# ywz978020607/MASIC

Measured on AMD Instinct MI355X. Metric: stereo pairs/sec (enc+dec), higher is better.
Workload: dtype bf16; 1 GPU; HSIC(N=128,M=192,K=5) eval forward (enc+dec both views), 8x3x512x512 stereo pairs per GPU (BASELINE.json configs[1] shape), inputs resident in HBM (the graph's static input buffers); the device homography of batch k+1 is handed over with batch k (one-batch look-ahead of a loader): its device->host read, the float32 host chain and the upload of the sampling matrices are done every step, under the r; pairs_per_gpu=8, height=512, width=512, parallelism=dp1 (pairs sharded, no data-path collective)

## Files before the change

coremasic/mywork/MASIC.py:

```python
import math
import os

import numpy as np

import torch
import torch.nn as nn
import torch.nn.functional as F

from compressai.entropy_models import (EntropyBottleneck, GaussianConditional, GaussianMixtureConditional,
                                       GaussianMixtureConditional_gf)
from compressai.layers import GDN, MaskedConv2d, ResidualBlock, conv3x3
from compressai.models.utils import conv, deconv, update_registered_buffers
from masic_amd import ops as _hip
from masic_amd.homography import warp_matrices as _warp_matrices
from masic_amd import autograd as _ag
from masic_amd.streams import ForkJoin as _ForkJoin
from masic_amd import fp8 as _fp8
from masic_amd import deconv as _deconv
from masic_amd.f16k import F16K as _F16K, F8K as _F8K

_RELU, _LEAKY, _NONE = _hip.ACT_RELU, _hip.ACT_LEAKY, _hip.ACT_NONE
_CAT_F16K = True
_HEADS_GROUPED = True


class CompressionModel(nn.Module):

    def __init__(self, entropy_bottleneck_channels, init_weights=True):
        super().__init__()
        self.entropy_bottleneck1 = EntropyBottleneck(entropy_bottleneck_channels)
        self.entropy_bottleneck2 = EntropyBottleneck(entropy_bottleneck_channels)
        if init_weights:
            self._initialize_weights()

    def aux_loss(self):
        return sum(m.loss() for m in self.modules() if isinstance(m, EntropyBottleneck))

    def _initialize_weights(self):
        for m in self.modules():
            if isinstance(m, (nn.Conv2d, nn.ConvTranspose2d)):
                nn.init.kaiming_normal_(m.weight)
                if m.bias is not None:
                    nn.init.zeros_(m.bias)

    def forward(self, *args):
        raise NotImplementedError()

    def parameters(self):
        for child in self.children():
            if not isinstance(child, EntropyBottleneck):
                yield from child.parameters()

    def aux_parameters(self):
        for child in self.children():
            if isinstance(child, EntropyBottleneck):
                yield from child.parameters()

    def update(self, force=False):
        for child in self.children():
            if isinstance(child, EntropyBottleneck):
                child.update(force=force)


class RateDistortionLoss(nn.Module):

    def __init__(self, lmbda=1e-2):
        super().__init__()
        self.lmbda = lmbda

    def forward(self, output, target):
        N, _, H, W = target.size()
        n = N * H * W
        bpp = sum(_hip.sum_log(l.contiguous()) for l in output["likelihoods"].values()) / (-math.log(2) * n)
        mse = _hip.sse(output["x_hat"].contiguous(), target.contiguous()) / target.numel()
        return {"bpp_loss": bpp.float(), "mse_loss": mse.float(), "loss": (self.lmbda * 255 ** 2 * mse + bpp).float()}


class AverageMeter:
    def __init__(self):
        self.val = self.avg = self.sum = self.count = 0

    def update(self, val, n=1):
        self.val = val
        self.sum += val * n
        self.count += n
        self.avg = self.sum / self.count


_SIDE_STREAMS = {}


def _side_streams(device, n=4):
    key = torch.device(device).index
    pool = _SIDE_STREAMS.get(key)
    if pool is None:
        pool, seen = [], set()
        for _ in range(64):
            s = torch.cuda.Stream(device=device)
            if s.cuda_stream not in seen:
                seen.add(s.cuda_stream)
                pool.append(s)
            if len(pool) == n + 1:
                break
        pool = _SIDE_STREAMS[key] = tuple(pool)
    cur = torch.cuda.current_stream(device).cuda_stream
    return tuple(s for s in pool if s.cuda_stream != cur)[:n]


_TRAIN_STREAMS = os.environ.get("MASIC_TRAIN_STREAMS", "1") != "0"


def _keep_until(t, stream):
    if not (torch.is_tensor(t) or isinstance(t, _F16K)):
        return
    if not torch.cuda.is_current_stream_capturing():
        t.record_stream(stream)


def _bf16_inference(*tensors):
    from masic_amd import nn as _mnn
    if not _mnn.reduced_precision():
        return False
    return not (torch.is_grad_enabled() and any(t.requires_grad for t in tensors))


def _f16k_chain(convs, acts, x, in_op=0, out=None, out_coff=0, gate=None, gate_c=0):
    B, _, H, W = x.shape
    hw = (H, W)
    for cv in convs:
        if not cv.f16k_supported(B, *hw):
            return None
        hw = cv.out_hw(*hw)
    t = x if isinstance(x, _F16K) else _F16K.from_nchw(x, in_op=in_op)
    for cv, act in zip(convs[:-1], acts):
        t = cv.run_f16k(t, act=act)
    return convs[-1].run_f16k(t, act=acts[-1], want_nchw=out is None, out=out, out_coff=out_coff, gate=gate, gate_c=gate_c)


def _pair_conv(conv, xa, xb, gdn_in=None, gdn_out=None):
    B, _, H, W = xa.shape
    desc = conv._desc((B, 6, H, W))
    def g(m):
        return None if m is None else (m.beta.detach(), m.gamma.detach().contiguous(), m.inverse)
    bm = (gdn_in or gdn_out).beta_min if (gdn_in or gdn_out) is not None else 1e-6
    return _hip.conv5s1_pair(xa, xb, conv.packed_weight(desc), None if conv.bias is None else conv.bias.detach(),
                             gdn_in=g(gdn_in), gdn_out=g(gdn_out), beta_min=bm)


def _gdn_f16k(gdn, x):
    return _hip.gdn_f16k(x, gdn.beta.detach(), gdn.gamma.detach(), inverse=gdn.inverse, beta_min=gdn.beta_min)


def _analysis_f16k(owner, x, layouts=None):
    from masic_amd import nn as _mnn
    convs = (owner.g_a_conv1, owner.g_a_conv2, owner.g_a_conv3, owner.g_a_conv4)
    gdns = (owner.g_a_gdn1, owner.g_a_gdn2, owner.g_a_gdn3)
    B, C, H, W = x.shape
    c1 = convs[0]
    if (C, c1.out_channels, tuple(c1.kernel_size), tuple(c1.stride), tuple(c1.padding)) != (3, 128, (5, 5), (2, 2), (2, 2)):
        return None
    sizes = [((H - 1) // 2 + 1, (W - 1) // 2 + 1)]
    for cv in convs[1:]:
        if not cv.f16k_supported(B, *sizes[-1]):
            return None
        sizes.append(cv.out_hw(*sizes[-1]))
    if convs[1].out_channels != 128 or convs[2].out_channels != 128:
        return None
    b1 = None if c1.bias is None else c1.bias.detach()
    sc = _fp8.scales(owner)
    if layouts is not None and (sc is not None or _mnn._FP8 or _fp8.recording() or not convs[3].f16k_multi_supported(B, *sizes[2])):
        return None
    if sc is not None and convs[1].f8k_supported(B, *sizes[0]) and convs[2].f8k_supported(B, *sizes[1]):
        t8 = _hip.conv_a_gdn_f8k(x, c1.packed_first_layer_weight(), b1, (_mnn.packed_gdn_f16k(gdns[0]), gdns[0].inverse), sc["a1"])[0]
        t = convs[1].run_f8k(_F8K(t8, B, 128, *sizes[0], sc["a1"]), gdn=gdns[1], out="f8k", out_scale=sc["a2"])
        t = convs[2].run_f8k(t, gdn=gdns[2], out="f16k")
        return convs[3].run_f16k(t, want_nchw=True)
    t = _F16K(_hip.conv_a_gdn_f16k(x, c1.packed_first_layer_weight(), b1, (_mnn.packed_gdn_f16k(gdns[0]), gdns[0].inverse))[0], B, 128, *sizes[0], 128, 0)
    _fp8.record(owner, "a1", t.buf)
    t = convs[1].run_f16k(t, gdn=gdns[1])
    _fp8.record(owner, "a2", t.buf)
    t = convs[2].run_f16k(t, gdn=gdns[2])
    if layouts is not None:
        return convs[3].run_f16k_multi(t, **layouts)
    return convs[3].run_f16k(t, want_nchw=True)


class encode_hyper(nn.Module):

    def __init__(self, N, M):
        super().__init__()
        self.encode_hyper = nn.Sequential(
            conv(M, N, kernel_size=5, stride=1), nn.ReLU(inplace=True),
            conv(N, N, kernel_size=5), nn.ReLU(inplace=True),
            conv(N, N, kernel_size=5))

    def forward(self, y, abs16=None):
        s = self.encode_hyper
        if _bf16_inference(y, s[0].weight):
            z = _f16k_chain((s[0], s[2], s[4]), (_RELU, _RELU, _NONE), y if abs16 is None else abs16, in_op=_hip.INOP_ABS)
            if z is not None:
                return z
        t = s[0].run(y, in_op=_hip.INOP_ABS, act=_RELU)
        t = s[2].run(t, act=_RELU)
        return s[4].run(t)


class _GmmHeads(nn.Module):

    def _branch(self, seq, x, acts):
        t = seq[0].run(x, act=acts[0])
        t = seq[2].run(t, act=acts[1])
        return seq[4].run(t, act=acts[2])

    def _branch_f16k(self, seq, x, acts):
        t, (B, _, H, W) = x.buf, x.shape
        for i, (layer, act) in enumerate(zip((seq[0], seq[2], seq[4]), acts)):
            last = i == 2
            if layer.in_channels % 16 == 0 and layer.out_channels % 32 == 0:
                t = _hip.gemm_f16k(t, layer.packed_gemm_dma_weight(), layer.bias.detach(), B, layer.in_channels, layer.out_channels,
                                   H, W, act, want_nchw=last)
            else:
                t = _hip.gemm1x1_bf16(t, layer.packed_gemm_weight(), layer.bias.detach(), B, layer.in_channels, layer.out_channels,
                                      H, W, act, want_nchw=last)
        return t

    def _branch_f8k(self, seq, x, sc, tag, acts):
        l0, l1, l2 = seq[0], seq[2], seq[4]
        x8, (B, _, H, W) = x.buf, x.shape
        wp, ws = l0.packed_gemm_f8k_weight(sc["c"])
        t = _hip.gemm_f8k(x8, wp, ws, l0.bias.detach(), B, l0.in_channels, l0.out_channels, H, W, acts[0], out="f8k", out_scale=sc[tag])
        wp, ws = l1.packed_gemm_f8k_weight(sc[tag])
        t = _hip.gemm_f8k(t, wp, ws, l1.bias.detach(), B, l1.in_channels, l1.out_channels, H, W, acts[1], out="f16k")
        return _hip.gemm_f16k(t, l2.packed_gemm_dma_weight(), l2.bias.detach(), B, l2.in_channels, l2.out_channels, H, W, acts[2], want_nchw=True)

    _STACKS = (("gmm_sigma", "h_sigma", (_RELU, _RELU, _RELU)), ("gmm_means", "h_means", (_LEAKY, _LEAKY, _NONE)),
               ("gmm_weights", "h_weights", (_LEAKY, _LEAKY, _NONE)))

    def _grouped_heads_ok(self):
        return all(getattr(self, n)[i].in_channels % 16 == 0 and getattr(self, n)[i].out_channels % 32 == 0
                   for n, _, _ in self._STACKS for i in (0, 2, 4))

    def _heads_grouped(self, x, sc):
        B, _, H, W = x.shape
        t = [x.buf] * 3
        for i in range(3):
            layers = []
            for k, (name, tag, acts) in enumerate(self._STACKS):
                layer = getattr(self, name)[2 * i]
                L = dict(x=t[k], bias=layer.bias.detach(), Cin=layer.in_channels, Cout=layer.out_channels, act=acts[i],
                         out="nchw" if i == 2 else "f16k")
                if sc is not None and i < 2:
                    L["wp"], L["ws"] = layer.packed_gemm_f8k_weight(sc["c"] if i == 0 else sc[tag])
                    if i == 0:
                        L["out"], L["out_scale"] = "f8k", sc[tag]
                else:
                    L["wp"] = layer.packed_gemm_dma_weight()
                layers.append(L)
            t = _hip.gemm_f16k_group(layers, B, H, W)
        return tuple(t)

    def _f8k_heads_ok(self):
        return all(seq[i].in_channels % 32 == 0 and seq[i].out_channels % 32 == 0 for seq in (self.gmm_sigma, self.gmm_means, self.gmm_weights) for i in (0, 2)) \
            and all(seq[4].in_channels % 16 == 0 and seq[4].out_channels % 32 == 0 for seq in (self.gmm_sigma, self.gmm_means, self.gmm_weights))

    def heads(self, x, parallel=True):
        from masic_amd import nn as _mnn
        if isinstance(x, _F16K):
            if not x.whole:
                raise RuntimeError(f"_GmmHeads.heads: the grouped GEMMs read a whole buffer, not {x!r}")
            return self._heads_grouped(x, None)
        if _mnn.reduced_precision() and not (torch.is_grad_enabled() and (x.requires_grad or self.gmm_sigma[0].weight.requires_grad)):
            B, _, H, W = x.shape
            sc = _fp8.scales(self)
            use_f8 = sc is not None and self._f8k_heads_ok()
            if use_f8:
                xv = _F8K(_hip.nchw_to_f8k(x, sc["c"]), *x.shape, sc["c"])
                branch = lambda seq, tag, acts: self._branch_f8k(seq, xv, sc, tag, acts)
            else:
                xv = _F16K.from_nchw(x)
                xf = xv.buf

                def branch(seq, tag, acts):
                    if _fp8.recording():
                        _fp8.record(self, "c", x)
                        l0 = seq[0]
                        _fp8.record(self, tag, _hip.gemm_f16k(xf, l0.packed_gemm_dma_weight(), l0.bias.detach(), B, l0.in_channels, l0.out_channels, H, W, acts[0])
                                    if l0.in_channels % 16 == 0 and l0.out_channels % 32 == 0 else
                                    _hip.gemm1x1_bf16(xf, l0.packed_gemm_weight(), l0.bias.detach(), B, l0.in_channels, l0.out_channels, H, W, acts[0]))
                    return self._branch_f16k(seq, xv, acts)
            if _HEADS_GROUPED and not _fp8.recording() and self._grouped_heads_ok():
                return self._heads_grouped(xv, sc if use_f8 else None)
            if not parallel:
                return (branch(self.gmm_sigma, "h_sigma", (_RELU, _RELU, _RELU)),
                        branch(self.gmm_means, "h_means", (_LEAKY, _LEAKY, _NONE)),
                        branch(self.gmm_weights, "h_weights", (_LEAKY, _LEAKY, _NONE)))
            fj = _ForkJoin()
            cur = fj.main
            side = _side_streams(x.device)[2:4]
            outs = [None, None, None]
            for i, (st, (seq, tag, acts)) in enumerate(zip(side, ((self.gmm_means, "h_means", (_LEAKY, _LEAKY, _NONE)),
                                                                  (self.gmm_weights, "h_weights", (_LEAKY, _LEAKY, _NONE))))):
                fj.fork(st)
                with fj.on(st):
                    outs[i + 1] = branch(seq, tag, acts)
            outs[0] = branch(self.gmm_sigma, "h_sigma", (_RELU, _RELU, _RELU))
            for st in side:
                fj.join(st)
            for t in outs[1:] + [xv.buf]:
                _keep_until(t, cur)
            return tuple(outs)
        if torch.is_grad_enabled() and _ag.gmm_heads_supported(self, x):
            return _ag.gmm_heads(self, x)
        sigma = self._branch(self.gmm_sigma, x, (_RELU, _RELU, _RELU))
        means = self._branch(self.gmm_means, x, (_LEAKY, _LEAKY, _NONE))
        logits = self._branch(self.gmm_weights, x, (_LEAKY, _LEAKY, _NONE))
        return sigma, means, logits

    def forward(self, x):
        sigma, means, logits = self.heads(x)
        return sigma, means, _hip.softmax_k(logits, self.K)


class gmm_hyper_y1_same_resolution(_GmmHeads):

    def __init__(self, N, M, K):
        super().__init__()
        self.N, self.M, self.K = N, M, K
        self.gmm_sigma = nn.Sequential(
            deconv(4 * M, 6 * M, kernel_size=1, stride=1), nn.ReLU(inplace=True),
            deconv(6 * M, 4 * M, kernel_size=1, stride=1), nn.ReLU(inplace=True),
            conv(4 * M, M * K, kernel_size=1, stride=1), nn.ReLU(inplace=True))
        self.gmm_means = nn.Sequential(
            deconv(4 * M, 6 * M, kernel_size=1, stride=1), nn.LeakyReLU(inplace=True),
            deconv(6 * M, 4 * M, kernel_size=1, stride=1), nn.LeakyReLU(inplace=True),
            conv(4 * M, M * K, kernel_size=1, stride=1))
        self.gmm_weights = nn.Sequential(
            deconv(4 * M, 6 * M, kernel_size=1, stride=1), nn.LeakyReLU(inplace=True),
            deconv(6 * M, M * K, kernel_size=1, stride=1), nn.LeakyReLU(inplace=True),
            conv(M * K, M * K, kernel_size=1, stride=1))


class gmm_hyper_y2_same_resolution(_GmmHeads):

    def __init__(self, N, M, K):
        super().__init__()
        self.N, self.M, self.K = N, M, K
        self.gmm_sigma = nn.Sequential(
            conv(5 * M, 6 * M, kernel_size=1, stride=1), nn.ReLU(inplace=True),
            conv(6 * M, 4 * M, kernel_size=1, stride=1), nn.ReLU(inplace=True),
            conv(4 * M, M * K, kernel_size=1, stride=1), nn.ReLU(inplace=True))
        self.gmm_means = nn.Sequential(
            conv(5 * M, 6 * M, kernel_size=1, stride=1), nn.LeakyReLU(inplace=True),
            conv(6 * M, 4 * M, kernel_size=1, stride=1), nn.LeakyReLU(inplace=True),
            conv(4 * M, M * K, kernel_size=1, stride=1))
        self.gmm_weights = nn.Sequential(
            conv(5 * M, 6 * M, kernel_size=1, stride=1), nn.LeakyReLU(inplace=True),
            conv(6 * M, M * K, kernel_size=1, stride=1), nn.LeakyReLU(inplace=True),
            conv(M * K, M * K, kernel_size=1, stride=1))


class mask2weights(nn.Module):

    def __init__(self, N, M, Kw):
        super().__init__()
        self.maskconv = nn.Sequential(
            conv(1, 3, kernel_size=3, stride=2), nn.ReLU(inplace=True),
            conv(3, 6, kernel_size=3), nn.ReLU(inplace=True),
            conv(6, 6, kernel_size=3), nn.ReLU(inplace=True),
            conv(6, 3, kernel_size=3))
        self.N, self.M, self.Kw = N, M, Kw

    def forward(self, m):
        s = self.maskconv
        t = s[0].run(m, act=_RELU)
        t = s[2].run(t, act=_RELU)
        t = s[4].run(t, act=_RELU)
        return s[6].run(t, act=_hip.ACT_SOFTMAX_C)


def _synthesis_f16k(dec, y_hat):
    B, _, H, W = y_hat.shape
    convs = (dec.g_s_conv1, dec.g_s_conv2, dec.g_s_conv3)
    gdns = (dec.g_s_gdn1, dec.g_s_gdn2, dec.g_s_gdn3)
    sizes = [(H, W)]
    for cv in convs:
        if cv.out_channels != 128 or not cv.f16k_supported(B, *sizes[-1]):
            return None
        sizes.append(cv.out_hw(*sizes[-1]))
    if not dec.g_s_conv4.d2s_supported(B, *sizes[3]):
        return None
    t = y_hat if isinstance(y_hat, _F16K) else _F16K.from_nchw(y_hat)
    sc = _fp8.scales(dec)
    if sc is not None and convs[1].f8k_supported(B, *sizes[1]) and convs[2].f8k_supported(B, *sizes[2]):
        t = convs[0].run_f16k_f8out(t, sc["d1"], gdn=gdns[0])
        t = convs[1].run_f8k(t, gdn=gdns[1], out="f8k", out_scale=sc["d2"])
        t = convs[2].run_f8k(t, gdn=gdns[2], out="f16k")
        return dec.g_s_conv4.run_f16k_d2s(t)
    for i in range(3):
        if t.whole and _deconv.supported(convs[i], gdns[i], B, t.H, t.W):
            t = _deconv.run(convs[i], gdns[i], t)
        else:
            t = convs[i].run_f16k(t, gdn=gdns[i])
        if i < 2:
            _fp8.record(dec, "d%d" % (i + 1), t.buf)
    return dec.g_s_conv4.run_f16k_d2s(t)


class Encoder1(nn.Module):

    def __init__(self, N, M, **kwargs):
        super().__init__()
        self.g_a_conv1 = conv(3, N)
        self.g_a_gdn1 = GDN(N)
        self.g_a_conv2 = conv(N, N)
        self.g_a_gdn2 = GDN(N)
        self.g_a_conv3 = conv(N, N)
        self.g_a_gdn3 = GDN(N)
        self.g_a_conv4 = conv(N, M)

    def forward(self, x):
        g1 = self.g_a_gdn1(self.g_a_conv1(x))
        g2 = self.g_a_gdn2(self.g_a_conv2(g1))
        g3 = self.g_a_gdn3(self.g_a_conv3(g2))
        return self.g_a_conv4(g3), g1, g2, g3

    def latent(self, x):
        if _bf16_inference(x, self.g_a_conv1.weight):
            y = _analysis_f16k(self, x.contiguous())
            if y is not None:
                return y
        return self.forward(x)[0]

    def latent_layouts(self, x, **layouts):
        if _bf16_inference(x, self.g_a_conv1.weight):
            return _analysis_f16k(self, x.contiguous(), layouts=layouts)
        return None

    def latent_train(self, x):
        if _ag.analysis_supported(self, x):
            return _ag.analysis(self, x)
        return self.forward(x)[0]


class Decoder1(nn.Module):

    def __init__(self, N, M, **kwargs):
        super().__init__()
        self.g_s_conv1 = deconv(M, N)
        self.g_s_gdn1 = GDN(N, inverse=True)
        self.g_s_conv2 = deconv(N, N)
        self.g_s_gdn2 = GDN(N, inverse=True)
        self.g_s_conv3 = deconv(N, N)
        self.g_s_gdn3 = GDN(N, inverse=True)
        self.g_s_conv4 = deconv(N, 3)

    def forward(self, y_hat):
        g1 = self.g_s_gdn1(self.g_s_conv1(y_hat))
        g2 = self.g_s_gdn2(self.g_s_conv2(g1))
        g3 = self.g_s_gdn3(self.g_s_conv3(g2))
        return self.g_s_conv4(g3), g1, g2, g3

    def reconstruct(self, y_hat):
        if isinstance(y_hat, _F16K):
            return _synthesis_f16k(self, y_hat) if _bf16_inference(self.g_s_conv1.weight) else None
        if _bf16_inference(y_hat, self.g_s_conv1.weight):
            x_hat = _synthesis_f16k(self, y_hat)
            if x_hat is not None:
                return x_hat
        return self.forward(y_hat)[0]

    def reconstruct_train(self, y_hat):
        if _ag.synthesis_supported(self, y_hat):
            return _ag.synthesis(self, y_hat)
        return self.forward(y_hat)[0]


class Encoder2(nn.Module):

    def __init__(self, N, M, **kwargs):
        super().__init__()
        self.pre_conv = conv(6, 3, stride=1)
        self.pre_gdn = GDN(3)
        self.g_a_conv1 = conv(3, N)
        self.g_a_gdn1 = GDN(N)
# ... 927 lines not shown
```

Measured before the change: 4415 stereo pairs/s.

## Add dedicated stride-2 128->128 5x5 conv+GDN kernel for encoder layers 2-3

Adds a specialized HIP kernel for the 128-channel 5x5 stride-2 conv fused with GDN. It splits waves into weight-DMA and patch-DMA roles, keeps a ring buffer of weight slabs in LDS, double-buffers input patches, and prefetches gamma for an in-register GDN epilogue. It also maps images to XCDs when the batch is divisible by 8. The encoder chain routes its two middle layers through this kernel when supported, aiming to hide load latency behind MFMA. The cost is a large, shape-specialized kernel with one block per CU, which limits occupancy.

```diff
diff --git a/coremasic/mywork/MASIC.py b/coremasic/mywork/MASIC.py
--- a/coremasic/mywork/MASIC.py
+++ b/coremasic/mywork/MASIC.py
@@ -17,6 +17,7 @@
 from masic_amd.streams import ForkJoin as _ForkJoin
 from masic_amd import fp8 as _fp8
 from masic_amd import deconv as _deconv
+from masic_amd import conv_s2 as _conv_s2
 from masic_amd.f16k import F16K as _F16K, F8K as _F8K
 
 _RELU, _LEAKY, _NONE = _hip.ACT_RELU, _hip.ACT_LEAKY, _hip.ACT_NONE
@@ -177,9 +178,13 @@
         return convs[3].run_f16k(t, want_nchw=True)
     t = _F16K(_hip.conv_a_gdn_f16k(x, c1.packed_first_layer_weight(), b1, (_mnn.packed_gdn_f16k(gdns[0]), gdns[0].inverse))[0], B, 128, *sizes[0], 128, 0)
     _fp8.record(owner, "a1", t.buf)
-    t = convs[1].run_f16k(t, gdn=gdns[1])
-    _fp8.record(owner, "a2", t.buf)
-    t = convs[2].run_f16k(t, gdn=gdns[2])
+    for i in (1, 2):
+        if t.whole and _conv_s2.supported(convs[i], gdns[i], B, t.H, t.W):
+            t = _conv_s2.run(convs[i], gdns[i], t)
+        else:
+            t = convs[i].run_f16k(t, gdn=gdns[i])
+        if i == 1:
+            _fp8.record(owner, "a2", t.buf)
     if layouts is not None:
         return convs[3].run_f16k_multi(t, **layouts)
     return convs[3].run_f16k(t, want_nchw=True)
diff --git a/include/masic_conv_s2.h b/include/masic_conv_s2.h
--- /dev/null
+++ b/include/masic_conv_s2.h
@@ -0,0 +1,21 @@
+#ifndef MASIC_CONV_S2_H
+#define MASIC_CONV_S2_H
+
+#include <stddef.h>
+
+#ifdef __cplusplus
+extern "C" {
+#endif
+
+int masic_conv_s2_gdn_f16k_supported(int B, int Hi, int Wi);
+
+int masic_conv_s2_gdn_f16k_fwd(const void* x_f16k, const void* w_packed, const float* bias, const void* gdn_packed, void* y_f16k,
+                               int B, int Hi, int Wi, void* stream);
+
+int masic_conv_s2_gdn_f16k_kernel_name(int B, int Hi, int Wi, char* buf, size_t n);
+
+#ifdef __cplusplus
+}
+#endif
+
+#endif
diff --git a/masic_amd/conv_s2.py b/masic_amd/conv_s2.py
--- /dev/null
+++ b/masic_amd/conv_s2.py
@@ -0,0 +1,96 @@
+import ctypes
+import os
+
+import torch
+
+from . import _lib, ops
+from .f16k import F16K
+from .ops import _p, _stream
+
+HEADER_PATH = os.path.join(os.path.dirname(_lib.HEADER_PATH), "masic_conv_s2.h")
+CHANNELS = 128
+PACKED_BYTES = 8 * 5 * 20480
+
+
+def _bind():
+    if not os.path.exists(HEADER_PATH):
+        raise ImportError(f"masic_amd.conv_s2: {HEADER_PATH} is missing: the binding is derived from it.  There is no CPU fallback for "
+                          "the HIP path.")
+    with open(HEADER_PATH) as f:
+        signatures, constants, structs = _lib.parse_header(f.read(), header="masic_conv_s2.h")
+    if constants or structs:
+        raise ValueError("masic_conv_s2.h: declares constants or structs; it holds prototypes only")
+    for name, (res, args) in signatures.items():
+        if not name.startswith("masic_conv_s2_") or name in _lib.SIGNATURES:
+            raise ValueError(f"masic_conv_s2.h: {name} is not a masic_conv_s2_* entry point of its own")
+        fn = getattr(_lib.lib, name)
+        fn.restype = res
+        fn.argtypes = args
+    return signatures
+
+
+SIGNATURES = _bind()
+
+
+def out_hw(Hi, Wi):
+    return (Hi - 1) // 2 + 1, (Wi - 1) // 2 + 1
+
+
+def kernel_name(B, Hi, Wi):
+    buf = ctypes.create_string_buffer(96)
+    _lib.check(_lib.lib.masic_conv_s2_gdn_f16k_kernel_name(B, Hi, Wi, buf, 96), "conv_s2_gdn_f16k_kernel_name")
+    return buf.value.decode()
+
+
+def conv_s2_gdn_f16k(x16, packed, bias, gdn_packed, B, Hi, Wi, out16=None):
+    if x16.dtype != torch.int16 or not x16.is_cuda or x16.numel() != B * CHANNELS * Hi * Wi:
+        raise RuntimeError(f"masic_amd.conv_s2_gdn_f16k: input must be an F16K int16 CUDA buffer of [{B},{CHANNELS},{Hi},{Wi}]")
+    if packed.dtype != torch.int16 or packed.numel() * 2 != PACKED_BYTES or packed.device != x16.device:
+        raise RuntimeError("masic_amd.conv_s2_gdn_f16k: `packed` is not the slab stream of a 128 -> 128 5x5 stride-2 layer")
+    if gdn_packed.numel() * gdn_packed.element_size() != ops._int_query("masic_gdn_f16k_packed_bytes") or gdn_packed.device != x16.device:
+        raise RuntimeError("masic_amd.conv_s2_gdn_f16k: `gdn_packed` is not a packed 128-channel GDN")
+    if bias is not None:
+        ops._dev(bias, "bias")
+        if bias.numel() != CHANNELS or bias.device != x16.device:
+            raise RuntimeError("masic_amd.conv_s2_gdn_f16k: bias must hold 128 values on the input's device")
+    if not _lib.lib.masic_conv_s2_gdn_f16k_supported(B, Hi, Wi):
+        raise RuntimeError(f"masic_amd.conv_s2_gdn_f16k: shape [{B},{CHANNELS},{Hi},{Wi}] is not supported")
+    Ho, Wo = out_hw(Hi, Wi)
+    n_out = B * CHANNELS * Ho * Wo
+    if out16 is None:
+        out16 = torch.empty(n_out, dtype=torch.int16, device=x16.device)
+    elif out16.dtype != torch.int16 or out16.numel() != n_out or out16.device != x16.device or not out16.is_contiguous():
+        raise RuntimeError("masic_amd.conv_s2_gdn_f16k: out16 does not match the output")
+    timed = None
+    if ops._timer is not None:
+        desc = ops.make_conv_desc(B, CHANNELS, Hi, Wi, CHANNELS, 5, 5, 2, 2, prec=_lib.PREC_BF16)
+        timed = ops._timer_open(desc, lambda d, buf, n: _lib.lib.masic_conv_s2_gdn_f16k_kernel_name(B, Hi, Wi, buf, n))
+    _lib.check(_lib.lib.masic_conv_s2_gdn_f16k_fwd(_p(x16), _p(packed), _p(bias), _p(gdn_packed), _p(out16), B, Hi, Wi, _stream()),
+               "conv_s2_gdn_f16k_fwd")
+    if timed is not None:
+        ops._timer_close(timed)
+    return out16
+
+
+def supported(cv, gdn, B, Hi, Wi, out_ctot=None, out_coff=0, in_ctot=None, in_coff=0, y_pre=None, prec=_lib.PREC_BF16, products=None):
+    if gdn is None or getattr(cv, "transposed_conv", True) or getattr(cv, "masked_conv", True):
+        return False
+    if cv.in_channels != CHANNELS or cv.out_channels != CHANNELS:
+        return False
+    if cv._geometry() != (5, 5, 2, 2) or gdn.inverse or gdn.beta.numel() != CHANNELS:
+        return False
+    if prec != _lib.PREC_BF16 or y_pre is not None or (ops._gdn_flags(False, products) & 2):
+        return False
+    if out_coff != 0 or out_ctot not in (None, CHANNELS) or in_coff != 0 or in_ctot not in (None, CHANNELS):
+        return False
+    return bool(_lib.lib.masic_conv_s2_gdn_f16k_supported(B, Hi, Wi)) and cv.f16k_supported(B, Hi, Wi)
+
+
+def run(cv, gdn, x):
+    from .nn import packed_gdn_f16k
+    if not x.whole or x.C != CHANNELS:
+        raise RuntimeError(f"masic_amd.conv_s2.run: the kernel takes whole 128-channel tensors, not {x!r}")
+    desc = cv._desc_f16k(x.B, x.H, x.W, out_ctot=CHANNELS)
+    bias = None if cv.bias is None else cv.bias.detach()
+    y16 = conv_s2_gdn_f16k(x.buf, cv.packed_f16k_weight(desc), bias, packed_gdn_f16k(gdn), x.B, x.H, x.W)
+    return F16K(y16, x.B, CHANNELS, desc.Ho, desc.Wo, CHANNELS, 0)
diff --git a/masic_amd/csrc/conv_s2_gdn.hip b/masic_amd/csrc/conv_s2_gdn.hip
--- /dev/null
+++ b/masic_amd/csrc/conv_s2_gdn.hip
@@ -0,0 +1,236 @@
+#include "f16k_device.h"
+#include "masic_conv_s2.h"
+
+namespace {
+
+struct ConvS2Args {
+    const unsigned short* x;
+    const unsigned char* w;
+    const float* bias;
+    const unsigned char* gdn;
+    unsigned short* y;
+    int Hi, Wi, Ho, Wo, tiles_w, ntiles, xcd_images;
+};
+
+constexpr int CS_T = 5, CS_D = 2, CS_NWS = CS_D + 1, CS_WST = CS_T * 4096;
+constexpr int CS_CHUNKS = 8, CS_STEPS = CS_CHUNKS * 5;
+constexpr int CS_TH = 8, CS_TW = 32;
+constexpr int CS_PH = (CS_TH - 1) * 2 + 5, CS_PW = (CS_TW - 1) * 2 + 5, CS_PWH = (CS_PW + 1) / 2;
+constexpr int CS_HALF = CS_PH * CS_PWH;
+constexpr int CS_NPIX = (2 * CS_HALF + 31) / 32 * 32;
+constexpr int CS_NINSTR = CS_NPIX / 32;
+constexpr int CS_PB = CS_NINSTR * 1024;
+constexpr int CS_PSP = 6, CS_NPI = 2 * CS_PSP;
+constexpr int CS_RING = 0, CS_PATCH0 = CS_RING + CS_NWS * CS_WST, CS_BETA = CS_PATCH0 + 2 * CS_PB, CS_BIAS = CS_BETA + 512;
+constexpr int CS_LDS = CS_BIAS + 512;
+constexpr int CS_OOB = 0x7ffffff0;
+static_assert(CS_LDS <= 160 * 1024, "LDS");
+static_assert(CS_NPI * 4 >= CS_NINSTR && (CS_NPI - 2) * 4 <= CS_NINSTR, "a surplus DMA slot repeats instruction 4 (NPI - 3) + wave of the chunk");
+static_assert(32 * 1024 + 4 * 1024 <= CS_PB && CS_NPI * 4 >= 32, "gamma^ and its surplus slots fit a patch buffer and the DMA slots of a chunk");
+
+constexpr int cs_tap(int tj) { return ((tj & 1) * CS_HALF + (tj >> 1)) * 16; }
+
+__global__ __launch_bounds__(512, 1) void conv_s2_gdn_f16k(const ConvS2Args a) {
+    extern __shared__ __attribute__((aligned(1024))) unsigned char lds[];
+    const unsigned ldsb = (unsigned)(size_t)(__attribute__((address_space(3))) unsigned char*)lds;
+
+    const int tid = threadIdx.x, lane = tid & 63;
+    const int wave = __builtin_amdgcn_readfirstlane(tid >> 6);
+    const int j = lane & 31, h = lane >> 5;
+    const bool wrole = wave < 4;
+    const int wq = wave & 3;
+
+    int tile, b;
+    if (a.xcd_images) {
+        const int idx = (blockIdx.x >> 3) + (gridDim.x >> 3) * blockIdx.z;
+        const int slot = idx / (int)gridDim.x;
+        tile = idx - slot * (int)gridDim.x;
+        b = slot * 8 + (blockIdx.x & 7);
+    } else {
+        tile = blockIdx.x;
+        b = blockIdx.z;
+    }
+    if (tile >= a.ntiles) return;
+    const int th_i = tile / a.tiles_w, tw_i = tile - th_i * a.tiles_w;
+    const int r0 = th_i * CS_TH, c0 = tw_i * CS_TW;
+    const int plane_bytes = a.Hi * a.Wi * 32;
+
+    const __amdgpu_buffer_rsrc_t rx = __builtin_amdgcn_make_buffer_rsrc((void*)(a.x + (size_t)b * 8 * (size_t)(a.Hi * a.Wi * 16)), 0, 8 * plane_bytes, 0x00020000);
+    const __amdgpu_buffer_rsrc_t rw = __builtin_amdgcn_make_buffer_rsrc((void*)a.w, 0, CS_STEPS * CS_WST, 0x00020000);
+    const __amdgpu_buffer_rsrc_t rg = __builtin_amdgcn_make_buffer_rsrc((void*)a.gdn, 0, 65536 + 512, 0x00020000);
+
+    int wsoff = 0;
+    if (wrole) {
+#pragma unroll
+        for (int d = 0; d < CS_D; ++d) {
+#pragma unroll
+            for (int k = 0; k < CS_T; ++k) dma_buf16(rw, lds + CS_RING + d * CS_WST + k * 4096 + wq * 1024, wq * 1024 + lane * 16, wsoff + k * 4096);
+            wsoff += CS_WST;
+        }
+    }
+
+    auto patch_instr = [&](int k) { return k * 4 + wq < CS_NINSTR ? k * 4 + wq : (CS_NPI - 3) * 4 + wq; };
+    int goff[CS_NPI];
+#pragma unroll
+    for (int k = 0; k < CS_NPI; ++k) {
+        const int q = patch_instr(k) * 64 + lane;
+        const int hh = q >= CS_NPIX ? 1 : 0, pp = q - hh * CS_NPIX;
+        const int par = pp >= CS_HALF ? 1 : 0, rem = pp - par * CS_HALF;
+        const int pr = rem / CS_PWH, pc = 2 * (rem - pr * CS_PWH) + par;
+        const int ih = 2 * r0 - 2 + pr, iw = 2 * c0 - 2 + pc;
+        const bool ok = pp < 2 * CS_HALF && pc < CS_PW && ih >= 0 && ih < a.Hi && iw >= 0 && iw < a.Wi;
+        goff[k] = ok ? (ih * a.Wi + iw) * 32 + hh * 16 : CS_OOB;
+    }
+
+    if (!wrole) {
+#pragma unroll
+        for (int k = 0; k < CS_NPI; ++k) dma_buf16(rx, lds + CS_PATCH0 + patch_instr(k) * 1024, goff[k], 0);
+    }
+    if (tid < 128) {
+        reinterpret_cast<float*>(lds + CS_BETA)[tid] = reinterpret_cast<const float*>(a.gdn + 65536)[tid];
+        reinterpret_cast<float*>(lds + CS_BIAS)[tid] = a.bias != nullptr ? a.bias[tid] : 0.0f;
+    }
+    asm volatile("s_waitcnt vmcnt(0)" ::: "memory");
+    __syncthreads();
+
+    f32x16 acc[4];
+    {
+        const float* bp = reinterpret_cast<const float*>(lds + CS_BIAS) + 4 * h;
+#pragma unroll
+        for (int m = 0; m < 4; ++m)
+#pragma unroll
+            for (int q = 0; q < 4; ++q) {
+                const float4 bv = *reinterpret_cast<const float4*>(bp + m * 32 + 8 * q);
+                acc[m][4 * q + 0] = bv.x; acc[m][4 * q + 1] = bv.y; acc[m][4 * q + 2] = bv.z; acc[m][4 * q + 3] = bv.w;
+            }
+#pragma unroll
+        for (int m = 0; m < 4; ++m) asm volatile("" : "+v"(acc[m]));
+    }
+
+    const int bl = (h * CS_NPIX + 2 * wave * CS_PWH + j) * 16;
+    const int al = (h * 128 + j) * 16;
+
+    int cslot = 0, pslot = (CS_D % CS_NWS) * CS_WST;
+    int cb = CS_PATCH0, pb = CS_PATCH0 + CS_PB;
+
+    auto step = [&](auto slice, int t, bool last, int xs, bool gam) {
+        constexpr int S = decltype(slice)::value;
+        const int wvo = wsoff < CS_STEPS * CS_WST ? wq * 1024 + lane * 16 : CS_OOB;
+        auto dma_pieces = [&](int first, int end) {
+            if (wrole) {
+#pragma unroll
+                for (int k = first; k < end; ++k)
+                    if (k < CS_T) dma_buf16(rw, lds + CS_RING + pslot + k * 4096 + wq * 1024, wvo, wsoff + k * 4096);
+            } else if (S >= 0) {
+#pragma unroll
+                for (int u = first; u < end; ++u) {
+                    constexpr int k0 = (S >= 0 ? S : 0) * CS_PSP;
+                    if (u < CS_PSP) {
+                        if (gam) {
+                            const int p = (k0 + u) * 4 + wq;
+                            dma_buf16(rg, lds + pb + (p < 32 ? p : 32 + wq) * 1024, p < 32 ? lane * 16 : CS_OOB, p < 32 ? p * 2048 : 0);
+                        } else {
+                            dma_buf16(rx, lds + pb + patch_instr(k0 + u) * 1024, goff[k0 + u], xs);
+                        }
+                    }
+                }
+            }
+        };
+        constexpr int NPIECES = CS_T > CS_PSP ? CS_T : CS_PSP, per = (NPIECES + CS_T - 1) / CS_T;
+        const unsigned wst = ldsb + CS_RING + al + cslot;
+        const unsigned pst = ldsb + cb + t * (CS_PWH * 16) + bl;
+        v4u af[2][4], bfr[2];
+        auto request = [&](auto ic, auto bc) {
+            constexpr int i = decltype(ic)::value, buf = decltype(bc)::value;
+            ds_read128<cs_tap(i)>(bfr[buf], pst);
+            static_for<0, 4>([&](auto mc) {
+                constexpr int m = decltype(mc)::value;
+                ds_read128<i * 4096 + m * 512>(af[buf][m], wst);
+            });
+        };
+        request(std::integral_constant<int, 0>{}, std::integral_constant<int, 0>{});
+        static_for<0, CS_T>([&](auto ic) {
+            constexpr int i = decltype(ic)::value, buf = i & 1;
+            if constexpr (i + 1 < CS_T) request(std::integral_constant<int, i + 1>{}, std::integral_constant<int, (i + 1) & 1>{});
+            constexpr int pending = i + 1 < CS_T ? 5 : 0;
+            lgkm_wait<pending>(bfr[buf], af[buf][0], af[buf][1], af[buf][2], af[buf][3]);
+            static_for<0, 4>([&](auto mc) {
+                constexpr int m = decltype(mc)::value;
+                acc[m] = __builtin_amdgcn_mfma_f32_32x32x16_bf16(__builtin_bit_cast(bf16x8, af[buf][m]), __builtin_bit_cast(bf16x8, bfr[buf]), acc[m], 0, 0, 0);
+            });
+            __builtin_amdgcn_sched_barrier(0);
+            dma_pieces(i * per, (i + 1) * per);
+            __builtin_amdgcn_sched_barrier(0);
+        });
+        if (wrole) {
+            wsoff += CS_WST;
+            pslot = pslot + CS_WST == CS_NWS * CS_WST ? 0 : pslot + CS_WST;
+        }
+        cslot = cslot + CS_WST == CS_NWS * CS_WST ? 0 : cslot + CS_WST;
+        if (wrole) asm volatile("s_waitcnt vmcnt(%0)" ::"n"((CS_D - 1) * CS_T) : "memory");
+        else if (last) asm volatile("s_waitcnt vmcnt(0)" ::: "memory");
+        __builtin_amdgcn_s_barrier();
+    };
+
+    for (int c = 0; c < CS_CHUNKS; ++c) {
+        const int xs = (c + 1) * plane_bytes;
+        const bool gam = c + 1 == CS_CHUNKS;
+        step(std::integral_constant<int, 0>{}, 0, false, xs, gam);
+        step(std::integral_constant<int, 1>{}, 1, false, xs, gam);
+        for (int t = 2; t < 5; ++t) step(std::integral_constant<int, -1>{}, t, t == 4, xs, gam);
+        const int tmp = cb; cb = pb; pb = tmp;
+    }
+    asm volatile("s_waitcnt vmcnt(0)" ::: "memory");
+
+    gdn_in_registers<false, 1024>(acc, lds + CS_PATCH0 + lane * 16, reinterpret_cast<const float*>(lds + CS_BETA) + 4 * h, 0);
+    const int r = r0 + wave, c = c0 + j;
+    if (r < a.Ho && c < a.Wo) {
+        const size_t oplane = (size_t)a.Ho * a.Wo;
+        const unsigned op16 = (unsigned)oplane * 16;
+        unsigned short* yb = a.y + (((size_t)b * 8) * oplane + (size_t)r * a.Wo + c) * 16 + 8 * h;
+#pragma unroll
+        for (int m = 0; m < 4; ++m) store_f16k_tile(acc[m], yb + (size_t)(2 * m) * op16, op16);
+    }
+}
+static_assert(CS_CHUNKS % 2 == 0, "the epilogue reads gamma^ from the first patch buffer");
+
+struct ConvS2Plan {
+    int Ho, Wo, tiles_w, ntiles, xcd_images;
+    dim3 grid;
+};
+
+bool conv_s2_shape_ok(int B, int Hi, int Wi) {
+    return B >= 1 && B <= 65535 && Hi >= 1 && Wi >= 1 && (long long)Hi * Wi * 256 < (1ll << 31);
+}
+
+ConvS2Plan conv_s2_plan(int B, int Hi, int Wi) {
+    ConvS2Plan p{};
+    p.Ho = (Hi - 1) / 2 + 1;
+    p.Wo = (Wi - 1) / 2 + 1;
+    p.tiles_w = ceil_div(p.Wo, CS_TW);
+    p.ntiles = p.tiles_w * ceil_div(p.Ho, CS_TH);
+    p.xcd_images = B % 8 == 0;
+    p.grid = dim3(round_up(p.ntiles, 8), 1, B);
+    return p;
+}
+
+}
+
+extern "C" int masic_conv_s2_gdn_f16k_supported(int B, int Hi, int Wi) { return conv_s2_shape_ok(B, Hi, Wi) ? 1 : 0; }
+
+extern "C" int masic_conv_s2_gdn_f16k_kernel_name(int B, int Hi, int Wi, char* buf, size_t n) {
+    MASIC_REQUIRE(buf && n > 0 && conv_s2_shape_ok(B, Hi, Wi), MASIC_ERR_ARG, "conv_s2_gdn_f16k_kernel_name: bad arguments");
+    MASIC_REQUIRE((size_t)snprintf(buf, n, "conv_s2_gdn_f16k") < n, MASIC_ERR_ARG, "conv_s2_gdn_f16k_kernel_name: buffer of %zu bytes too small", n);
+    return MASIC_OK;
+}
+
+extern "C" int masic_conv_s2_gdn_f16k_fwd(const void* x_f16k, const void* w_packed, const float* bias, const void* gdn_packed, void* y_f16k,
+                                          int B, int Hi, int Wi, void* stream) {
+    MASIC_REQUIRE(x_f16k && w_packed && gdn_packed && y_f16k, MASIC_ERR_ARG, "conv_s2_gdn_f16k_fwd: null pointer");
+    MASIC_REQUIRE(conv_s2_shape_ok(B, Hi, Wi), MASIC_ERR_UNSUPPORTED, "conv_s2_gdn_f16k_fwd: %d x %d x %d is not supported", B, Hi, Wi);
+    const ConvS2Plan p = conv_s2_plan(B, Hi, Wi);
+    const ConvS2Args a{(const unsigned short*)x_f16k, (const unsigned char*)w_packed, bias, (const unsigned char*)gdn_packed, (unsigned short*)y_f16k,
+                       Hi, Wi, p.Ho, p.Wo, p.tiles_w, p.ntiles, p.xcd_images};
+    launch_lds<conv_s2_gdn_f16k>(p.grid, 512, CS_LDS, (hipStream_t)stream, a);
+    return masic_launch_status("conv_s2_gdn_f16k_fwd");
+}
```

Measured after the change: 4501 stereo pairs/s (median of 6 runs). +2.0%, better.
